# montib/rays1bench

Measured on AMD Instinct MI355X. Metric: mrays/s on 'large' scene 1200x800x10spp, higher is better.
Workload: dtype f32

## Files before the change

### rays1bench_amd/csrc/r1_builds.h

```cpp
#ifndef R1_BUILDS_H
#define R1_BUILDS_H

constexpr int R1_V_REFERENCE = 1;
constexpr int R1_V_SWEEP = 2;
constexpr int R1_V_SWEEP_STATS = 3;
constexpr int R1_V_TREE = 4;
constexpr int R1_V_TREE_STATS = 5;
constexpr int R1_V_WAVEFRONT = 6;
constexpr int R1_V_GRID = 7;
constexpr int R1_V_GRID_STATS = 8;

constexpr int R1_MODE_TP = 0;
constexpr int R1_MODE_LAT = 1;
constexpr int R1_MODE_PIXEL = 2;
constexpr int R1_MODE_BATCH = 3;
constexpr int R1_MODE_PASS = 4;
constexpr int R1_MODE_PATH = 5;
constexpr int R1_MODE_LISTED = 6;
constexpr int R1_MODES = 7;

constexpr bool r1_is_tree(int variant) { return variant == R1_V_TREE || variant == R1_V_TREE_STATS; }
constexpr bool r1_is_grid(int variant) { return variant == R1_V_GRID || variant == R1_V_GRID_STATS; }
constexpr bool r1_is_stats(int variant) { return variant == R1_V_SWEEP_STATS || variant == R1_V_TREE_STATS || variant == R1_V_GRID_STATS; }
constexpr int r1_base_variant(int variant) { return r1_is_stats(variant) ? variant - 1 : variant; }

constexpr bool r1_mode_is_batch(int mode) { return mode == R1_MODE_BATCH || mode == R1_MODE_PATH; }
constexpr bool r1_mode_is_pass(int mode) { return mode == R1_MODE_PASS || mode == R1_MODE_LISTED; }
constexpr bool r1_mode_is_tp_family(int mode) { return mode == R1_MODE_TP || r1_mode_is_batch(mode); }
constexpr bool r1_runs_as_latency(int mode, bool big) { return mode == R1_MODE_LAT || (r1_mode_is_pass(mode) && !big); }
constexpr bool r1_build_lands(int variant, bool stats, int mode) { return variant == R1_V_TREE && !stats && r1_mode_is_tp_family(mode); }

constexpr bool r1_root_by_slots(bool stats, bool big, int mode)
{
    return stats || (mode != R1_MODE_PATH && !(mode == R1_MODE_PIXEL && !big));
}

struct R1Build
{
    int variant;
    bool stats, big;
    int mode;
};

#define R1_BUILDS_TREE_SMALL(X)                 \
    X(R1_V_TREE, false, false, R1_MODE_TP)      \
    X(R1_V_TREE, false, false, R1_MODE_LAT)     \
    X(R1_V_TREE, false, false, R1_MODE_PIXEL)   \
    X(R1_V_TREE, false, false, R1_MODE_BATCH)   \
    X(R1_V_TREE, false, false, R1_MODE_PASS)    \
    X(R1_V_TREE, false, false, R1_MODE_PATH)    \
    X(R1_V_TREE, false, false, R1_MODE_LISTED)  \
    X(R1_V_TREE, true, false, R1_MODE_LAT)
#define R1_BUILDS_TREE_BIG(X)                  \
    X(R1_V_TREE, false, true, R1_MODE_TP)      \
    X(R1_V_TREE, false, true, R1_MODE_PIXEL)   \
    X(R1_V_TREE, false, true, R1_MODE_BATCH)   \
    X(R1_V_TREE, false, true, R1_MODE_PASS)    \
    X(R1_V_TREE, false, true, R1_MODE_PATH)    \
    X(R1_V_TREE, false, true, R1_MODE_LISTED)  \
    X(R1_V_TREE, true, true, R1_MODE_TP)
#define R1_BUILDS_SWEEP_SMALL(X)                   \
    X(R1_V_SWEEP, false, false, R1_MODE_TP)        \
    X(R1_V_SWEEP, false, false, R1_MODE_LAT)       \
    X(R1_V_SWEEP, false, false, R1_MODE_PIXEL)     \
    X(R1_V_SWEEP, false, false, R1_MODE_BATCH)     \
    X(R1_V_SWEEP, false, false, R1_MODE_PASS)      \
    X(R1_V_SWEEP, false, false, R1_MODE_PATH)      \
    X(R1_V_SWEEP, false, false, R1_MODE_LISTED)    \
    X(R1_V_SWEEP, true, false, R1_MODE_LAT)        \
    X(R1_V_REFERENCE, false, false, R1_MODE_TP)    \
    X(R1_V_REFERENCE, false, false, R1_MODE_PASS)
#define R1_BUILDS_SWEEP_BIG(X)   \
    X(R1_V_SWEEP, false, true, R1_MODE_TP)                                         \
    X(R1_V_SWEEP, false, true, R1_MODE_PIXEL)                                      \
    X(R1_V_SWEEP, false, true, R1_MODE_BATCH)                                      \
    X(R1_V_SWEEP, false, true, R1_MODE_PASS)                                       \
    X(R1_V_SWEEP, false, true, R1_MODE_PATH)                                       \
    X(R1_V_SWEEP, false, true, R1_MODE_LISTED)                                     \
    X(R1_V_REFERENCE, false, true, R1_MODE_TP)                                     \
    X(R1_V_REFERENCE, false, true, R1_MODE_PASS)
#define R1_BUILDS_GRID_SMALL(X)                 \
    X(R1_V_GRID, false, false, R1_MODE_TP)      \
    X(R1_V_GRID, false, false, R1_MODE_LAT)     \
    X(R1_V_GRID, false, false, R1_MODE_BATCH)   \
    X(R1_V_GRID, false, false, R1_MODE_PASS)    \
    X(R1_V_GRID, false, false, R1_MODE_PATH)    \
    X(R1_V_GRID, false, false, R1_MODE_LISTED)  \
    X(R1_V_GRID, true, false, R1_MODE_LAT)
#define R1_BUILDS_GRID_BIG(X)                  \
    X(R1_V_GRID, false, true, R1_MODE_TP)      \
    X(R1_V_GRID, false, true, R1_MODE_PIXEL)   \
    X(R1_V_GRID, false, true, R1_MODE_BATCH)   \
    X(R1_V_GRID, false, true, R1_MODE_PASS)    \
    X(R1_V_GRID, false, true, R1_MODE_PATH)    \
    X(R1_V_GRID, false, true, R1_MODE_LISTED)  \
    X(R1_V_GRID, true, true, R1_MODE_TP)
#define R1_BUILDS_ALL(X) R1_BUILDS_TREE_SMALL(X) R1_BUILDS_TREE_BIG(X) R1_BUILDS_SWEEP_SMALL(X) R1_BUILDS_SWEEP_BIG(X) R1_BUILDS_GRID_SMALL(X) R1_BUILDS_GRID_BIG(X)

constexpr bool r1_same_build(const R1Build &a, int variant, bool stats, bool big, int mode)
{
    return a.variant == variant && a.stats == stats && a.big == big && a.mode == mode;
}

constexpr bool r1_build_exists(const R1Build &b)
{
#define R1_X(V, S, B, M) || r1_same_build(b, V, S, B, M)
    return false R1_BUILDS_ALL(R1_X);
#undef R1_X
}

constexpr bool r1_pick(int variant, bool big, int want, R1Build &b)
{
    if (variant < R1_V_REFERENCE || variant > R1_V_GRID_STATS || variant == R1_V_WAVEFRONT || want < 0 || want >= R1_MODES)
        return false;
    const bool single = want == R1_MODE_TP || want == R1_MODE_LAT || want == R1_MODE_PIXEL;
    b.variant = r1_base_variant(variant), b.stats = r1_is_stats(variant), b.big = big, b.mode = want;
    if (b.stats)
    {
        if (!single)
            return false;
        b.mode = big ? R1_MODE_TP : R1_MODE_LAT;
        if (b.variant == R1_V_SWEEP && big)
            b.stats = false;
    }
    else if (variant == R1_V_REFERENCE)
    {
        if (!single && want != R1_MODE_PASS)
            return false;
        b.mode = single ? R1_MODE_TP : R1_MODE_PASS;
    }
    else
    {
        if (want == R1_MODE_LAT && big)
            b.mode = R1_MODE_TP;
        if (variant == R1_V_GRID && want == R1_MODE_PIXEL && !big)
            return false;
    }
    return true;
}

constexpr bool r1_picks_exist()
{
    for (int variant = 0; variant <= 9; ++variant)
        for (int big = 0; big < 2; ++big)
            for (int want = 0; want < R1_MODES; ++want)
            {
                R1Build b = {0, false, false, 0};
                if (r1_pick(variant, big != 0, want, b) && !r1_build_exists(b))
                    return false;
            }
    return true;
}
static_assert(r1_picks_exist(), "r1_pick chose a build that no translation unit instantiates (R1_BUILDS_*)");

#endif
```

### rays1bench_amd/csrc/r1_hit_tree.hpp

```cpp
#ifndef R1_HIT_TREE_HPP
#define R1_HIT_TREE_HPP

#include <hip/hip_runtime.h>
#include <float.h>
#include <stdint.h>

#include "r1_device.h"
#include "r1_exact_math.h"
#include "r1_offer.h"
#include "r1_dev_math.hpp"

#pragma clang fp contract(off)

namespace
{

#define R1_BVH_DONE 0xFFFFFFFFu

__device__ __forceinline__ bool bvh_box(const float mx, const float my, const float mz, const float ex, const float ey, const float ez,
                                        const V3 pa, const V3 oi, const V3 inv, const V3 ainv, const float best, float &t_near)
{
    const float ax = __fmaf_rn(mx, inv.x, -oi.x), ay = __fmaf_rn(my, inv.y, -oi.y), az = __fmaf_rn(mz, inv.z, -oi.z);
    const float bx = __fmaf_rn(ex, ainv.x, pa.x), by = __fmaf_rn(ey, ainv.y, pa.y), bz = __fmaf_rn(ez, ainv.z, pa.z);
    const float tn = fmaxf(fmaxf(ax - bx, ay - by), az - bz);
    const float tf = fminf(fminf(ax + bx, ay + by), az + bz);
    t_near = tn;
    return tn <= tf && tn <= best && tf >= 0.0f;
}

template <int OFFER>
__device__ __forceinline__ void leaf_quad(const float4 *__restrict__ prims, const uint32_t *__restrict__ ids, const uint32_t first,
                                          const uint32_t pairs, const V3 o, const V3 d, float &best, uint32_t &best_id)
{
    float nb[4], ds[4];
#pragma unroll
    for (int h = 0; h < 2; ++h)
    {
        if (h)
            __builtin_amdgcn_sched_barrier(0);
        const float4 p0 = prims[2 * (size_t)first + 2 * h], p1 = prims[2 * (size_t)first + 2 * h + 1];
#pragma unroll
        for (int s = 0; s < 2; ++s)
        {
            const int q = 2 * h + s;
            const float cx = s ? p0.y : p0.x, cy = s ? p0.w : p0.z, cz = s ? p1.y : p1.x, rsq = s ? p1.w : p1.z;
            const float cox = cx - o.x, coy = cy - o.y, coz = cz - o.z;
            nb[q] = __fmaf_rn(coz, d.z, __fmaf_rn(coy, d.y, cox * d.x));
            const float c = __fmaf_rn(coz, coz, __fmaf_rn(coy, coy, cox * cox)) - rsq;
            ds[q] = nb[q] * nb[q] - c;
        }
    }
    uint32_t sgn = __float_as_uint(ds[3]) >> 31;
    sgn = __builtin_amdgcn_alignbit(sgn, __float_as_uint(ds[2]), 31u);
    sgn = __builtin_amdgcn_alignbit(sgn, __float_as_uint(ds[1]), 31u);
    sgn = __builtin_amdgcn_alignbit(sgn, __float_as_uint(ds[0]), 31u);
    uint32_t mask = ~sgn & (pairs < 2u ? 3u : 15u);
    unsigned long long flagged = __builtin_amdgcn_ballot_w64(mask != 0u);
    if (flagged != 0ull)
    do
    {
        const bool have = mask != 0u;
        const uint32_t q = (uint32_t)__builtin_ctz(mask | 8u);
        mask &= mask - 1u;
        const float n_ = q == 0u ? nb[0] : (q == 1u ? nb[1] : (q == 2u ? nb[2] : nb[3]));
        const float d_ = q == 0u ? ds[0] : (q == 1u ? ds[1] : (q == 2u ? ds[2] : ds[3]));
        const uint32_t id = ids[2 * (size_t)first + q];
        const float root = r1_sqrt_exact_lanes(d_, flagged);
        const float t1 = n_ - root;
        const float t = (t1 > 0.001f) ? t1 : n_ + root;
        const bool upd = have & r1_offer_update_form<OFFER>(t, id, best, best_id);
        best = upd ? t : best;
        best_id = upd ? id : best_id;
        flagged = __builtin_amdgcn_ballot_w64(mask != 0u);
    } while (flagged != 0ull);
}

template <int OFFER>
__device__ __forceinline__ void leaf_root(const float4 *__restrict__ prims, const uint32_t *__restrict__ ids, const uint32_t first,
                                          const uint32_t pairs, const V3 o, const V3 d, float &best, uint32_t &best_id)
{
    typedef const uint32_t __attribute__((address_space(4))) *cu32_ptr;
    const cf4_ptr sp = (cf4_ptr)(const f4 *)prims + 2 * (size_t)first;
    const cu32_ptr si = (cu32_ptr)ids + 2 * (size_t)first;
#pragma unroll
    for (int h = 0; h < 2; ++h)
    {
        if (h && pairs < 2u)
            break;
        const f4 p0 = sp[2 * h], p1 = sp[2 * h + 1];
#pragma unroll
        for (int s = 0; s < 2; ++s)
        {
            const float cx = s ? p0.y : p0.x, cy = s ? p0.w : p0.z, cz = s ? p1.y : p1.x, rsq = s ? p1.w : p1.z;
            const float cox = cx - o.x, coy = cy - o.y, coz = cz - o.z;
            const float nb = __fmaf_rn(coz, d.z, __fmaf_rn(coy, d.y, cox * d.x));
            const float c = __fmaf_rn(coz, coz, __fmaf_rn(coy, coy, cox * cox)) - rsq;
            const float ds = nb * nb - c;
            const unsigned long long any = __builtin_amdgcn_ballot_w64((int)__float_as_uint(ds) >= 0);
            if (any != 0ull)
            {
                const bool flag = (int)__float_as_uint(ds) >= 0;
                const uint32_t id = si[2 * h + s];
                const float root = r1_sqrt_exact_lanes(ds, any);
                const float t1 = nb - root;
                const float t = (t1 > 0.001f) ? t1 : nb + root;
                const bool upd = flag & r1_offer_update_form<OFFER>(t, id, best, best_id);
                best = upd ? t : best;
                best_id = upd ? id : best_id;
            }
        }
    }
}

__device__ __forceinline__ void trav_put(uint32_t *trav, const int at, const uint32_t ref) { trav[at] = ref; }
__device__ __forceinline__ uint32_t trav_get(const uint32_t *trav, const int at) { return trav[at]; }
__device__ __forceinline__ void trav_put(uint16_t *trav, const int at, const uint32_t ref) { trav[at] = (uint16_t)ref; }
__device__ __forceinline__ uint32_t trav_get(const uint16_t *trav, const int at) { return trav[at]; }
__device__ __forceinline__ uint32_t r1_ref16(const uint32_t ref) { return ((ref >> 16) & 0xF000u) | (ref & 0x0FFFu); }

struct Trav
{
    uint32_t cur;
    int sp;
    float best;
    uint32_t best_id;
};

__device__ __forceinline__ void trav_start(Trav &t)
{
    t.cur = 0u, t.sp = 0, t.best = FLT_MAX, t.best_id = 0xFFFFFFFFu;
}

#ifndef R1_CARRY_DIV
#define R1_CARRY_DIV 6u
#endif
template <bool STATS, bool CARRY, bool LN, typename TS, bool SLOTS = false, int OFFER = R1_OFFER_FORM>
__device__ __forceinline__ void bvh_advance(const R1DeviceScene &S, const V3 o, const V3 d, Trav &tv, TS *trav, const int tid,
                                            const uint32_t n_alive, unsigned long long *wstat, const float4 *lnodes , const uint32_t top = 0u )
{
    const float4 *__restrict__ nodes = S.bvh_nodes;
    const float4 *__restrict__ prims = S.bvh_prims;
    const uint32_t *__restrict__ ids = S.bvh_ids;
    const V3 inv = mk(__builtin_amdgcn_rcpf(d.x), __builtin_amdgcn_rcpf(d.y), __builtin_amdgcn_rcpf(d.z));
    const V3 ainv = mk(fabsf(inv.x), fabsf(inv.y), fabsf(inv.z));
    V3 oi = mk(o.x * inv.x, o.y * inv.y, o.z * inv.z);
    const float rx = o.x - S.bvh_centre[0], ry = o.y - S.bvh_centre[1], rz = o.z - S.bvh_centre[2];
    const float r2 = __fmaf_rn(rz, rz, __fmaf_rn(ry, ry, rx * rx));
    V3 pa_ray = mk(0.0f, 0.0f, 0.0f);
    if (LN)
    {
        const float pad_ray = lnodes[3].x * r2;
        pa_ray = mk(pad_ray * ainv.x, pad_ray * ainv.y, pad_ray * ainv.z);
    }
    float best = tv.best;
    uint32_t best_id = tv.best_id;
    uint32_t cur = tv.cur;
    int sp = tv.sp;
    constexpr uint32_t LEAF_BIT = LN ? 0x8000u : 0x80000000u, INDEX_MASK = LN ? 0x0FFFu : 0x0FFFFFFFu;
    constexpr int COUNT_SHIFT = LN ? 12 : 28;
    auto visit_node = [&]() {
        if (STATS)
        {
            wstat[9] += 1;
            if ((tid & 63) == __ffsll((long long)__ballot(1)) - 1)
                wstat[2] += 1;
        }
        float4 q0, q1, q2, q3;
        if (LN || cur < top)
        {
            q0 = lnodes[4 * cur + 0], q1 = lnodes[4 * cur + 1], q2 = lnodes[4 * cur + 2], q3 = lnodes[4 * cur + 3];
            if (!LN)
                asm volatile("" : "+v"(q0.x), "+v"(q1.x), "+v"(q2.x), "+v"(q3.x));
        }
        else
            q0 = nodes[4 * (size_t)cur + 0], q1 = nodes[4 * (size_t)cur + 1], q2 = nodes[4 * (size_t)cur + 2],
            q3 = nodes[4 * (size_t)cur + 3];
        float tn0, tn1;
        V3 pa = pa_ray;
        if (!LN)
        {
            float dist2 = r2;
            if (S.bvh_pad_local)
            {
                const float sx = __fmaf_rn(-2.0f, o.x, q0.x + q0.y), sy = __fmaf_rn(-2.0f, o.y, q0.z + q0.w), sz = __fmaf_rn(-2.0f, o.z, q1.x + q1.y);
                dist2 = __fmaf_rn(sz, sz, __fmaf_rn(sy, sy, sx * sx));
            }
            const float pad = __fmaf_rn(q3.x, dist2, q3.y);
            pa = mk(pad * ainv.x, pad * ainv.y, pad * ainv.z);
        }
        const bool h0 = bvh_box(q0.x, q0.z, q1.x, q1.z, q2.x, q2.z, pa, oi, inv, ainv, best, tn0);
        const bool h1 = bvh_box(q0.y, q0.w, q1.y, q1.w, q2.y, q2.w, pa, oi, inv, ainv, best, tn1);
        const uint32_t c0 = __float_as_uint(q3.z), c1 = __float_as_uint(q3.w);
        if (h0 && h1)
        {
            const bool swap = tn1 < tn0;
            trav_put(trav, sp * R1_BLOCK + tid, swap ? c0 : c1);
            ++sp;
            cur = swap ? c1 : c0;
        }
        else if (h0)
            cur = c0;
        else if (h1)
            cur = c1;
        else if (sp > 0)
            cur = trav_get(trav, --sp * R1_BLOCK + tid);
        else
            cur = R1_BVH_DONE;
    };
    auto visit_flat = [&]() {
        if (STATS)
        {
            wstat[9] += 1;
            if ((tid & 63) == __ffsll((long long)__ballot(1)) - 1)
                wstat[2] += 1;
        }
        const float4 q0 = lnodes[4 * cur + 0], q1 = lnodes[4 * cur + 1], q2 = lnodes[4 * cur + 2], q3 = lnodes[4 * cur + 3];
        const float ax0 = __fmaf_rn(q0.x, inv.x, -oi.x), az0 = __fmaf_rn(q1.x, inv.z, -oi.z);
        const float bx0 = __fmaf_rn(q1.z, ainv.x, pa_ray.x), bz0 = __fmaf_rn(q2.z, ainv.z, pa_ray.z);
        const float ax1 = __fmaf_rn(q0.y, inv.x, -oi.x), az1 = __fmaf_rn(q1.y, inv.z, -oi.z);
        const float bx1 = __fmaf_rn(q1.w, ainv.x, pa_ray.x), bz1 = __fmaf_rn(q2.w, ainv.z, pa_ray.z);
        const float tn0 = fmaxf(fmaxf(ax0 - bx0, az0 - bz0), oi.y), tf0 = fminf(fminf(ax0 + bx0, az0 + bz0), pa_ray.y);
        const float tn1 = fmaxf(fmaxf(ax1 - bx1, az1 - bz1), oi.y), tf1 = fminf(fminf(ax1 + bx1, az1 + bz1), pa_ray.y);
        const bool h0 = tn0 <= tf0, h1 = tn1 <= tf1;
        const uint32_t c0 = __float_as_uint(q3.z), c1 = __float_as_uint(q3.w);
        if (h0 && h1)
        {
            const bool swap = tn1 < tn0;
            trav_put(trav, sp * R1_BLOCK + tid, swap ? c0 : c1);
            ++sp;
            cur = swap ? c1 : c0;
        }
        else if (h0)
            cur = c0;
        else if (h1)
            cur = c1;
        else if (sp > 0)
            cur = trav_get(trav, --sp * R1_BLOCK + tid);
        else
            cur = R1_BVH_DONE;
    };
    const uint32_t root_leaf = LN ? __float_as_uint(lnodes[3].y) & 3u : S.bvh_root_leaf;
    if (root_leaf != 0u && cur == 0u)
    {
        const int k = root_leaf == 1u ? 1 : 0;
        const float *nf = (const float *)lnodes;
        const uint32_t leaf = __float_as_uint(nf[14 + (1 - k)]);
        const uint32_t other = __float_as_uint(nf[14 + k]);
        const uint32_t lp = (leaf >> COUNT_SHIFT) & 7u;
        if (STATS)
        {
            wstat[5] += (unsigned long long)lp, wstat[16] += 1ull, wstat[17] += 1ull;
            if ((tid & 63) == __ffsll((long long)__ballot(1)) - 1)
                wstat[3] += 1;
        }
        if (SLOTS)
            leaf_root<OFFER>(prims, ids, (uint32_t)__builtin_amdgcn_readfirstlane((int)(leaf & INDEX_MASK)), (uint32_t)__builtin_amdgcn_readfirstlane((int)lp), o, d, best, best_id);
        else
            leaf_quad<OFFER>(prims, ids, leaf & INDEX_MASK, lp, o, d, best, best_id);
        V3 pa = pa_ray;
        if (!LN)
        {
            float dist2 = r2;
            if (S.bvh_pad_local)
            {
                const float sx = __fmaf_rn(-2.0f, o.x, nf[0] + nf[1]), sy = __fmaf_rn(-2.0f, o.y, nf[2] + nf[3]), sz = __fmaf_rn(-2.0f, o.z, nf[4] + nf[5]);
                dist2 = __fmaf_rn(sz, sz, __fmaf_rn(sy, sy, sx * sx));
            }
            const float pad = __fmaf_rn(nf[12], dist2, nf[13]);
            pa = mk(pad * ainv.x, pad * ainv.y, pad * ainv.z);
        }
        float tn;
        const bool h = bvh_box(nf[0 + k], nf[2 + k], nf[4 + k], nf[6 + k], nf[8 + k], nf[10 + k], pa, oi, inv, ainv, best, tn);
        cur = h ? other : R1_BVH_DONE;
    }
    if (LN && (__builtin_amdgcn_readfirstlane((int)__float_as_uint(lnodes[3].y)) & 4) != 0)
    {
        const float a_u = __fmaf_rn(lnodes[7].x, inv.y, -oi.y), b_u = __fmaf_rn(lnodes[7].y, ainv.y, pa_ray.y);
        const float tyf = a_u + b_u;
        oi.y = fmaxf(a_u - b_u, 0.0f);
        pa_ray.y = tyf < best ? tyf : best;
        cur = oi.y <= pa_ray.y ? cur : R1_BVH_DONE;
    }
    for (;;)
    {
        const unsigned long long walking = __ballot(cur != R1_BVH_DONE);
        if (walking == 0ull)
            break;
        if (CARRY && R1_CARRY_DIV * (uint32_t)__popcll(walking) <= n_alive)
            break;
        if (LN && (__builtin_amdgcn_readfirstlane((int)__float_as_uint(lnodes[3].y)) & 4) != 0)
            while (cur < LEAF_BIT)
                visit_flat();
        else
            while (cur < LEAF_BIT)
                visit_node();
        if (cur != R1_BVH_DONE)
        {
            const uint32_t first = cur & INDEX_MASK, cnt = (cur >> COUNT_SHIFT) & 7u;
            if (LN)
            {
                static_assert(R1_BVH_LEAF <= 4, "the LDS walks test a leaf with ONE leaf_quad call: at most two pairs");
                if (STATS)
                {
                    wstat[5] += (unsigned long long)cnt, wstat[16] += 1ull;
                    if ((tid & 63) == __ffsll((long long)__ballot(1)) - 1)
                        wstat[3] += 1;
                }
                leaf_quad<OFFER>(prims, ids, first, cnt, o, d, best, best_id);
            }
            else
            for (uint32_t j = 0; j < cnt; j += 2u)
            {
                const uint32_t take = cnt - j < 2u ? 1u : 2u;
                if (STATS)
                {
                    wstat[5] += (unsigned long long)take;
                    wstat[16] += 1ull;
                    if ((tid & 63) == __ffsll((long long)__ballot(1)) - 1)
                        wstat[3] += 1;
                }
                leaf_quad<OFFER>(prims, ids, first + j, take, o, d, best, best_id);
            }
            cur = sp > 0 ? trav_get(trav, --sp * R1_BLOCK + tid) : R1_BVH_DONE;
            if (LN && (__builtin_amdgcn_readfirstlane((int)__float_as_uint(lnodes[3].y)) & 4) != 0)
                pa_ray.y = best < pa_ray.y ? best : pa_ray.y;
        }
    }
    tv.cur = cur, tv.sp = sp, tv.best = best, tv.best_id = r1_offer_settle_form<OFFER>(best, best_id);
}

template <bool STATS>
__device__ __forceinline__ void sweep_bvh(const R1DeviceScene &S, const bool alive, const V3 o, const V3 d, float &t_max, int &hit_index,
                                          uint32_t *trav, const int tid, unsigned long long *wstat)
{
    Trav tv;
    trav_start(tv);
    if (!alive)
        tv.cur = R1_BVH_DONE;
    bvh_advance<STATS, false, false, uint32_t>(S, o, d, tv, trav, tid, 64u, wstat, nullptr);
    if (tv.best_id != 0xFFFFFFFFu)
    {
        t_max = tv.best;
        hit_index = (int)tv.best_id;
    }
}

}

#endif
```

### rays1bench_amd/csrc/r1_trace.hpp

```cpp
#ifndef R1_TRACE_HPP
#define R1_TRACE_HPP

#include <hip/hip_runtime.h>
#include <float.h>
#include <stdint.h>

#include "r1_device.h"
#include "r1_dev_math.hpp"
#include "r1_kargs.hpp"
#include "r1_hit_sweep.hpp"
#include "r1_hit_tree.hpp"
#include "r1_hit_grid.hpp"
#include "r1_sample.hpp"
#include "r1_shade.hpp"
#include "r1_land.hpp"

#pragma clang fp contract(off)

template <int VARIANT, bool STATS, bool BIG, int MODE>
struct TraceWaves
{
#ifndef R1_TREE_WAVES_TP
#define R1_TREE_WAVES_TP 7
#endif
#ifndef R1_TREE_WAVES_LAT
#define R1_TREE_WAVES_LAT 6
#endif
    static constexpr int value = STATS ? 1 : (VARIANT == R1_V_GRID && MODE == R1_MODE_PIXEL) ? 4 : ((r1_is_tree(VARIANT) || r1_is_grid(VARIANT)) ? (BIG ? 8 : (r1_mode_is_tp_family(MODE) ? R1_TREE_WAVES_TP : R1_TREE_WAVES_LAT)) : (VARIANT == R1_V_SWEEP && !BIG ? 5 : 1));
};

template <int VARIANT, bool STATS, bool BIG, int MODE>
__device__ __forceinline__ void r1_trace_body(const R1TraceArgs A)
{
    constexpr bool LISTED = MODE == R1_MODE_LISTED, PASS = r1_mode_is_pass(MODE);
    constexpr bool CPATH = MODE == R1_MODE_PATH, BATCH = r1_mode_is_batch(MODE);
    constexpr bool LAT = r1_runs_as_latency(MODE, BIG), PIX = MODE == R1_MODE_PIXEL;
    constexpr bool LAND = r1_build_lands(VARIANT, STATS, MODE);
    const uint32_t tb = blockIdx.x, n_tb = gridDim.x;
    const uint32_t xcd = LAND ? (uint32_t)__builtin_amdgcn_readfirstlane((int)(xcc_id() & (R1_LAND_MAX_XCD - 1u))) : 0u;
    const uint32_t land_tiles = LAND ? A.total_samples / A.full : 0u;
#ifdef R1_LAND_DEBUG
    if (LAND && threadIdx.x == 0 && blockIdx.x < 8)
        A.queue[R1_HEAD_WORDS * (R1_HEAD_DEBUG + blockIdx.x % R1_HEAD_DEBUG_COUNT)] = 0x1000u | (xcc_id() << 4) | xcd;
#endif
    if (LAND && blockIdx.x == 0)
        for (uint32_t i = threadIdx.x; i < R1_HEAD_WORDS * A.land.clear_count; i += R1_BLOCK)
            A.land.clear_heads[i] = 0u;
    typedef typename IdxType<BIG>::type IDX;
    unsigned long long wstat[18];
    if (STATS)
    {
        for (int i = 0; i < 18; ++i)
            wstat[i] = 0;
        wstat[14] = __builtin_readcyclecounter();
    }
    unsigned long long *wave_log = nullptr;
    unsigned long long log_start = 0, log_exhausted = 0;
    if (STATS && A.stats)
    {
        wave_log = (unsigned long long *)A.stats[R1_STATS_WORDS];
        log_start = __builtin_amdgcn_s_memrealtime();
    }
    constexpr int LW = (r1_is_tree(VARIANT) || r1_is_grid(VARIANT)) ? ((r1_mode_is_tp_family(MODE) && !STATS) ? R1_STACK_LDS_WORDS_TP : R1_STACK_LDS_WORDS) : R1_STACK_WORDS;
    __shared__ uint32_t s_stack[BIG ? 1 : LW * R1_BLOCK];
    __shared__ uint32_t s_cand[VARIANT == R1_V_SWEEP ? (BIG ? R1_CAND_CAP : R1_BIT_WORDS) * R1_BLOCK : 1];
    __shared__ IDX s_pairs[VARIANT == R1_V_SWEEP ? (R1_BLOCK / 64) * PairBits<IDX>::cap : 1];
    extern __shared__ uint32_t s_trav[];
    const uint32_t gstride = n_tb * R1_BLOCK, gtid = tb * R1_BLOCK + threadIdx.x;
    __shared__ unsigned long long s_best[VARIANT == R1_V_SWEEP ? R1_BLOCK : 1];
    __shared__ f4 s_tile[BIG && VARIANT == R1_V_SWEEP ? 2 * R1_TILE_F4 : 1];

    const int tid = (int)threadIdx.x;
    const int lane = tid & 63;

    constexpr bool LN = VARIANT == R1_V_TREE && !BIG;
    typedef typename IdxType<!LN>::type TS;
    const size_t trav_words = VARIANT == R1_V_TREE ? (size_t)A.bvh_depth * R1_BLOCK * sizeof(TS) / 4 : 0;
    const size_t gtrav_words = VARIANT == R1_V_GRID ? (size_t)A.bvh_depth * R1_BLOCK : 0;
    const uint16_t *ltab = (const uint16_t *)(s_trav + gtrav_words);
    if (VARIANT == R1_V_GRID && !BIG)
    {
        float4 *dst = (float4 *)(s_trav + gtrav_words);
        const R1GridCArgs *ga = (const R1GridCArgs *)(uintptr_t)A.grid;
        const float4 *src = (const float4 *)(const r1_gu32 *)ga->tab;
        const uint32_t n16 = ga->lds_bytes / 16u;
        for (uint32_t i = (uint32_t)tid; i < n16; i += R1_BLOCK)
            dst[i] = src[i];
        __syncthreads();
    }
    const float4 *lnodes = (const float4 *)(s_trav + trav_words);
    const uint32_t top = LN ? 0u : A.bvh_lds_f4 >> 2;
    if (VARIANT == R1_V_TREE && A.bvh_lds_f4)
    {
        float4 *dst = (float4 *)(s_trav + trav_words);
        for (uint32_t i = (uint32_t)tid; i < A.bvh_lds_f4; i += R1_BLOCK)
        {
            float4 q = A.scene.bvh_nodes[i];
            if (LN && (i & 3u) == 3u)
                q.z = __uint_as_float(r1_ref16(__float_as_uint(q.z))), q.w = __uint_as_float(r1_ref16(__float_as_uint(q.w)));
            dst[i] = q;
        }
        if (LN && tid == 3)
            ((float *)dst)[13] = __uint_as_float(A.scene.bvh_root_leaf | (A.scene.bvh_flat_e >= 0.0f ? 4u : 0u));
        if (LN && tid == 7 && A.scene.bvh_flat_e >= 0.0f)
            ((float *)dst)[28] = A.scene.bvh_flat_m, ((float *)dst)[29] = A.scene.bvh_flat_e;
        __syncthreads();
    }

    Path p;
    p.o = mk(0, 0, 0), p.d = mk(0, 0, 0);
    p.s_scalar = p.s0 = p.s1 = p.s2 = 1;
    p.k = 0, p.depth = 0, p.sp = 0;
    bool alive = false;
    Pixel px;
    px.acc = mk(0, 0, 0), px.xy = 0, px.off = 0, px.s = (uint32_t)A.spp;
    Trav tv;
    trav_start(tv);
    tv.cur = R1_BVH_DONE;
    unsigned long long lane_rays = 0;
#ifndef R1_SPARE_MIN
#define R1_SPARE_MIN 40u
#endif
    constexpr bool SPARE = !BIG && (VARIANT == R1_V_TREE || VARIANT == R1_V_SWEEP || VARIANT == R1_V_GRID) && r1_mode_is_tp_family(MODE);
    Path spare = p;
    bool has_spare = false;
    constexpr bool TRIM = LAND && SPARE;
#ifndef R1_TRIM_VOTES
#define R1_TRIM_VOTES 1
#endif
#ifndef R1_TRIM_WALK
#define R1_TRIM_WALK 1
#endif
    constexpr bool TRIM_VOTES = TRIM && R1_TRIM_VOTES, TRIM_WALK = TRIM && R1_TRIM_WALK;
#define R1_DEAD (TRIM_VOTES ? tv.cur == R1_BVH_DONE : !alive)
#define R1_VOTE(c) (TRIM_VOTES ? (unsigned long long)__builtin_amdgcn_ballot_w64(c) : (unsigned long long)__ballot(c))

    uint32_t q_next = 0, q_end = 0;
    const uint32_t q_total = A.total_samples;
    uint32_t q_remaining = q_total;
    const uint32_t n_waves2 = 2u * n_tb * (R1_BLOCK / 64);
    uint32_t *const q_head = LAND ? A.queue + R1_HEAD_WORDS * (R1_HEAD_XCD + xcd) : A.queue;
    constexpr uint32_t LAND_GROUP = LAT ? 8u : 1u;
    __shared__ uint32_t s_land[LAND ? (R1_BLOCK / 64) * R1_LAND_ROW : 1];
#define row (s_land + (LAND ? (threadIdx.x >> 6) * R1_LAND_ROW : 0u))
    if (LAND && lane < 8)
        row[lane] = (lane == 0 || lane == 2) ? 0xFFFFFFFFu : 0u;
    bool exhausted = false;
    const uint32_t home = LAT && A.nq > 1 ? __builtin_amdgcn_readfirstlane(((tb >> 3) * (R1_BLOCK / 64) + (threadIdx.x >> 6)) % A.nq) : 0u;

    for (;;)
    {
        if (STATS)
            wstat[15] = __builtin_readcyclecounter();
        if (PIX && !alive && px.s < (uint32_t)A.spp)
        {
            start_ray(A, A.cam, p, (int)(px.xy & 0xFFFFu), (int)(px.xy >> 16), px.s, A.seed);
            alive = true;
            if (VARIANT == R1_V_TREE)
                trav_start(tv);
        }
        if (SPARE && R1_DEAD && has_spare)
        {
            p.o = spare.o, p.d = spare.d, p.s_scalar = spare.s_scalar, p.s0 = spare.s0, p.s1 = spare.s1, p.s2 = spare.s2, p.k = spare.k;
            p.depth = 0, p.sp = 0;
            alive = true, has_spare = false;
            if (TRIM_WALK)
                tv.cur = 0u;
            else
                trav_start(tv);
        }
        unsigned long long need = R1_VOTE(R1_DEAD);
        if (SPARE)
        {
            const unsigned long long lack = R1_VOTE(!has_spare);
            const uint32_t n_lack = TRIM_VOTES ? (uint32_t)__builtin_popcount((uint32_t)lack) + (uint32_t)__builtin_popcount((uint32_t)(lack >> 32)) : (uint32_t)__popcll(lack);
            need = (need != 0ull || n_lack >= R1_SPARE_MIN) ? lack : 0ull;
        }
        while (need)
        {
            if (q_next == q_end)
            {
                if (exhausted)
                    break;
                uint32_t want, base = 0;
                if (LAT && A.nq > 1)
                {
                    want = A.chunk_max;
                    if (lane == 0)
                        base = atomicAdd(A.queue + R1_HEAD_WORDS * (R1_HEAD_SUBQUEUE + home), 1u);
                    base = (__builtin_amdgcn_readfirstlane(base) * A.nq + home) * want;
                }
                else if (LAND)
                {
                    want = min(A.chunk_max, max(A.chunk_min, q_remaining / n_waves2));
                    base = q_total;
                    for (;;)
                    {
                        unsigned long long old = 0;
                        if (lane == 0)
                            old = __hip_atomic_fetch_add((unsigned long long *)q_head, (unsigned long long)want, __ATOMIC_RELAXED, __HIP_MEMORY_SCOPE_AGENT);
                        const uint32_t hi = (uint32_t)__builtin_amdgcn_readfirstlane((int)(uint32_t)(old >> 32));
                        const uint32_t lo = (uint32_t)__builtin_amdgcn_readfirstlane((int)(uint32_t)old);
                        if (hi == 0xFFFFFFFFu)
                            break;
                        const uint32_t g0 = (hi - 1u) * LAND_GROUP;
                        const uint32_t gs = hi != 0u ? min(LAND_GROUP, land_tiles - g0) * A.full : 0u;
                        const bool have = hi != 0u && lo < gs;
                        const bool advance = (hi == 0u && lo == 0u) || (have && lo + want >= gs);
                        if (advance && lane == 0)
                        {
                            const uint32_t g = __hip_atomic_fetch_add(A.queue + R1_HEAD_WORDS * R1_HEAD_DISPENSER, 1u, __ATOMIC_RELAXED, __HIP_MEMORY_SCOPE_AGENT);
                            unsigned long long nv = 0xFFFFFFFFull << 32;
                            if (g * LAND_GROUP < land_tiles)
                                nv = (unsigned long long)(g + 1u) << 32;
                            (void)__hip_atomic_exchange((unsigned long long *)q_head, nv, __ATOMIC_RELAXED, __HIP_MEMORY_SCOPE_AGENT);
                        }
                        if (have)
                        {
                            base = g0 * A.full + lo;
                            want = min(want, gs - lo);
                            q_remaining = (land_tiles - min(land_tiles, g0 + LAND_GROUP)) * A.full;
                            const uint32_t tl = fastdiv(lo, A.div_full);
                            if (lane == 0)
                            {
                                land_chunk(A, row, g0 + tl);
                                if (lo - tl * A.full + want > A.full)
                                    land_chunk(A, row, g0 + tl + 1u);
                            }
                            break;
                        }
                        if (advance)
                            continue;
                        for (;;)
                        {
                            __builtin_amdgcn_s_sleep(16);
                            unsigned long long now = 0;
                            if (lane == 0)
                                now = __hip_atomic_load((unsigned long long *)q_head, __ATOMIC_RELAXED, __HIP_MEMORY_SCOPE_AGENT);
                            if ((uint32_t)__builtin_amdgcn_readfirstlane((int)(uint32_t)(now >> 32)) != hi)
                                break;
                        }
                    }
                }
                else
                {
                    want = min(A.chunk_max, max(A.chunk_min, q_remaining / n_waves2));
                    if (lane == 0)
                        base = atomicAdd(q_head, want);
                    base = __builtin_amdgcn_readfirstlane(base);
                }
                if (base >= q_total)
                {
                    exhausted = true;
                    if (STATS)
                        log_exhausted = __builtin_amdgcn_s_memrealtime();
                    break;
                }
                q_next = base;
                q_end = min(base + want, q_total);
                if (!LAND)
                    q_remaining = q_total - q_end;
            }
            const uint32_t avail = q_end - q_next;
            const uint32_t rank = __builtin_amdgcn_mbcnt_hi((uint32_t)(need >> 32), __builtin_amdgcn_mbcnt_lo((uint32_t)need, 0u));
            R1ArgWords FA_words;
            if (!PIX)
                fresh_args(FA_words);
            const R1TraceArgs &FA = PIX ? A : FA_words.a;
            if (SPARE)
            {
                if (!has_spare && rank < avail)
                    has_spare = start_sample<BATCH, PASS, CPATH, LISTED>(FA, spare, q_next + rank);
            }
            else if (!alive && rank < avail)
            {
                if (PIX)
                {
                    alive = pixel_take(A, px, q_next + rank);
                    if (alive)
                        start_ray(A, A.cam, p, (int)(px.xy & 0xFFFFu), (int)(px.xy >> 16), 0u, A.seed);
                }
                else
                    alive = start_sample<BATCH, PASS, CPATH, LISTED>(FA, p, q_next + rank);
                if (VARIANT == R1_V_TREE && alive)
                    trav_start(tv);
            }
            q_next += min((uint32_t)__popcll(need), avail);
            need = SPARE ? R1_VOTE(!has_spare) : R1_VOTE(!alive);
        }
        if (SPARE && R1_DEAD && has_spare)
        {
            p.o = spare.o, p.d = spare.d, p.s_scalar = spare.s_scalar, p.s0 = spare.s0, p.s1 = spare.s1, p.s2 = spare.s2, p.k = spare.k;
            p.depth = 0, p.sp = 0;
            alive = true, has_spare = false;
            if (TRIM_WALK)
                tv.cur = 0u;
            else
                trav_start(tv);
        }
        if (BIG && VARIANT == R1_V_SWEEP)
        {
            if (!__syncthreads_or(alive ? 1 : 0))
                break;
        }
        else if (!TRIM_VOTES && __ballot(alive) == 0ull)
            break;
        if (TRIM_VOTES)
            alive = !R1_DEAD;
        const unsigned long long live_once = TRIM_VOTES ? (unsigned long long)__builtin_amdgcn_ballot_w64(!R1_DEAD) : 0ull;
        if (TRIM_VOTES && live_once == 0ull)
            break;
        if (TRIM_VOTES)
        {
            if ((__builtin_amdgcn_ballot_w64(p.depth >= 12) & live_once) == 0ull)
                __builtin_amdgcn_s_setprio(0);
            else if ((__builtin_amdgcn_ballot_w64(p.depth >= 36) & live_once) != 0ull)
                __builtin_amdgcn_s_setprio(3);
            else if ((__builtin_amdgcn_ballot_w64(p.depth >= 24) & live_once) != 0ull)
                __builtin_amdgcn_s_setprio(2);
            else
                __builtin_amdgcn_s_setprio(1);
        }
        else
        {
            if (__ballot(alive && p.depth >= 12) == 0ull)
                __builtin_amdgcn_s_setprio(0);
            else if (__ballot(alive && p.depth >= 36) != 0ull)
                __builtin_amdgcn_s_setprio(3);
            else if (__ballot(alive && p.depth >= 24) != 0ull)
                __builtin_amdgcn_s_setprio(2);
            else
                __builtin_amdgcn_s_setprio(1);
        }
        if (STATS)
        {
            wstat[4] += __builtin_readcyclecounter() - wstat[15];
            wstat[15] = __builtin_readcyclecounter();
            wstat[0] += 1;
            wstat[1] += (unsigned long long)__popcll(__ballot(alive));
        }

        float t_hit = FLT_MAX;
        int hit = -1;
        bool ready = alive;
        const unsigned long long live_now = TRIM_VOTES ? live_once : __ballot(alive);
        if (LAT && !BIG && VARIANT != R1_V_REFERENCE && exhausted && (uint32_t)__popcll(live_now) <= A.coop_lanes)
        {
            cooperative_sweep(A.scene, live_now, p.o, p.d, t_hit, hit, lane);
            tv.cur = R1_BVH_DONE;
        }
        else if (VARIANT == R1_V_REFERENCE)
        {
            if (alive)
                sweep_reference(A.scene, p.o, p.d, t_hit, hit);
        }
        else if (VARIANT == R1_V_TREE)
        {
            R1_FRESH_ARGS(HA)
            bvh_advance<STATS, true, LN, TS, r1_root_by_slots(STATS, BIG, MODE)>(HA.scene, p.o, p.d, tv, (TS *)s_trav, tid, (uint32_t)__popcll(live_now), wstat, lnodes, top);
            ready = alive && tv.cur == R1_BVH_DONE;
            if (tv.best_id != 0xFFFFFFFFu)
                t_hit = tv.best, hit = (int)tv.best_id;
        }
        else if (VARIANT == R1_V_GRID)
        {
            R1_FRESH_ARGS(HA)
            float best;
            uint32_t best_id;
            const bool fb = grid_trace<STATS, !BIG>(HA, (R1GridCArgs *)(uintptr_t)HA.grid, alive, p.o, p.d, best, best_id, ltab, tid, wstat);
            if (STATS)
                wstat[16] += fb ? 1ull : 0ull;
            if (__ballot(fb) != 0ull)
            {
                Trav fv;
                trav_start(fv);
                fv.best = best, fv.best_id = best_id;
                if (!fb)
                    fv.cur = R1_BVH_DONE;
                bvh_advance<false, false, false, uint32_t, false, R1_OFFER_FORM_GRID>(HA.scene, p.o, p.d, fv, s_trav, tid, 64u, wstat, nullptr);
                best = fv.best, best_id = fv.best_id;
            }
            if (best_id != 0xFFFFFFFFu)
                t_hit = best, hit = (int)best_id;
        }
        else
        {
            R1ArgWords HA_words;
            if (!PIX)
                fresh_args(HA_words);
            const R1TraceArgs &HA = PIX ? A : HA_words.a;
            sweep_prefilter<STATS, IDX, BIG>(HA.scene, alive, p.o, p.d, t_hit, hit, s_cand, s_pairs, s_best, s_tile, tid, wstat);
        }
        if (STATS)
        {
            wstat[6] += __builtin_readcyclecounter() - wstat[15];
            wstat[15] = __builtin_readcyclecounter();
        }

        bool fin = false;
        R1ArgWords SA_words;
        if (!PIX)
            fresh_args(SA_words);
        const R1TraceArgs &SA = PIX ? A : SA_words.a;
        if (ready)
        {
            V3 col;
            if (shade_level<BIG, LW>(SA, p, hit, t_hit, s_stack, gstride, gtid, tid, col))
            {
                if (PIX)
                {
                    px.acc = vadd(px.acc, col);
                    if (++px.s == (uint32_t)SA.spp)
                        pixel_write(SA, px);
                }
                else if (LAND)
                    SA.samples[p.k] = make_float4(col.x, col.y, col.z, __uint_as_float(path_rays(p) | SA.land_tag));
                else
                    SA.samples[p.k] = make_float4(col.x, col.y, col.z, __uint_as_float(path_rays(p)));
                if (!LAND)
                    lane_rays += path_rays(p);
                alive = false, fin = true;
            }
            else if (VARIANT == R1_V_TREE && !TRIM_WALK)
                trav_start(tv);
            if (TRIM_WALK)
            {
                trav_start(tv);
                if (fin)
                    tv.cur = R1_BVH_DONE;
            }
        }
        if (LAND && fin)
            land_count(SA, row, p.k);
        if (STATS)
            wstat[7] += __builtin_readcyclecounter() - wstat[15];
    }
    if (STATS)
    {
        wstat[8] = __builtin_readcyclecounter() - wstat[14];
        unsigned long long c9 = wstat[9];
        for (int off = 32; off > 0; off >>= 1)
            c9 += __shfl_down(c9, off, 64);
        wstat[9] = c9;
        if (VARIANT == R1_V_TREE || VARIANT == R1_V_GRID)
        {
            const int slots[5] = {2, 3, 5, 16, 17};
            for (int q = 0; q < 5; ++q)
            {
                unsigned long long c = wstat[slots[q]];
                for (int off = 32; off > 0; off >>= 1)
                    c += __shfl_down(c, off, 64);
                wstat[slots[q]] = c;
            }
        }
        if (lane == 0 && wave_log)
        {
            unsigned long long *rec = wave_log + 4 * (size_t)(blockIdx.x * (R1_BLOCK / 64) + (threadIdx.x >> 6));
            if (VARIANT == R1_V_GRID)
            {
                typedef unsigned long long __attribute__((address_space(1))) gu64;
                gu64 *grec = (gu64 *)(uintptr_t)rec;
                grec[0] = log_start, grec[1] = log_exhausted, grec[2] = __builtin_amdgcn_s_memrealtime(), grec[3] = wstat[0];
            }
            else
                rec[0] = log_start, rec[1] = log_exhausted, rec[2] = __builtin_amdgcn_s_memrealtime(), rec[3] = wstat[0];
        }
        if (lane == 0 && A.stats)
        {
            for (int i = 0; i < 10; ++i)
                atomicAdd(&A.stats[i], wstat[i]);
            atomicMax(&A.stats[10], wstat[8]);
            atomicMax(&A.stats[11], ~wstat[8]);
            atomicMax(&A.stats[12], (unsigned long long)__builtin_readcyclecounter());
            atomicMax(&A.stats[13], ~wstat[14]);
            if (VARIANT == R1_V_TREE || VARIANT == R1_V_GRID)
            {
                atomicAdd(&A.stats[14], wstat[16]);
                atomicAdd(&A.stats[15], wstat[17]);
            }
        }
    }

    if (LAND)
        land_exit<(BIG && VARIANT == R1_V_TREE) ? 6 : R1_LAND_LOADS>(A, row, lane);
#undef row
#undef R1_VOTE
#undef R1_DEAD
    if (!LAND)
    {
        for (int off = 32; off > 0; off >>= 1)
            lane_rays += __shfl_down(lane_rays, off, 64);
        if (lane == 0 && lane_rays)
            atomicAdd(A.num_rays, lane_rays);
    }
}

template <int VARIANT, bool STATS, bool BIG, int MODE>
__global__ void __launch_bounds__(R1_BLOCK, (TraceWaves<VARIANT, STATS, BIG, MODE>::value)) r1_trace_kernel(const R1TraceArgs A)
{
    r1_trace_body<VARIANT, STATS, BIG, MODE>(A);
}

template <bool STATS, bool BIG, int MODE>
__global__ void __launch_bounds__(R1_BLOCK, (TraceWaves<R1_V_GRID, STATS, BIG, MODE>::value)) r1_grid_kernel(const R1TraceArgs A)
{
    r1_trace_body<R1_V_GRID, STATS, BIG, MODE>(A);
}

template <int VARIANT, bool BIG>
__global__ void __launch_bounds__(R1_BLOCK, (TraceWaves<VARIANT, false, BIG, R1_MODE_PASS>::value)) r1_pass_kernel(const R1TraceArgs A)
{
    r1_trace_body<VARIANT, false, BIG, R1_MODE_PASS>(A);
}

template <int VARIANT, bool BIG>
__global__ void __launch_bounds__(R1_BLOCK, (TraceWaves<VARIANT, false, BIG, R1_MODE_PASS>::value)) r1_adaptive_kernel(const R1TraceArgs A)
{
    r1_trace_body<VARIANT, false, BIG, R1_MODE_LISTED>(A);
}

template <int VARIANT, bool BIG>
__global__ void __launch_bounds__(R1_BLOCK, (TraceWaves<VARIANT, false, BIG, R1_MODE_PATH>::value)) r1_path_kernel(const R1TraceArgs A)
{
    r1_trace_body<VARIANT, false, BIG, R1_MODE_PATH>(A);
}

#endif
```

Before: 44140.

## Add vote-driven BVH walk choosing node or leaf steps per wave

Adds a voted traversal loop for the tree walker. Each iteration the wave ballots how many lanes sit on inner nodes versus leaves and picks a node step or a leaf step by a weighted majority rule, instead of draining all inner nodes before any lane tests leaves. It is enabled by default only for big TP/batch builds. The goal is to cut SIMD divergence where lanes idle while others finish node walks, at the cost of two extra ballots per step and a carry-exit check that now runs only after leaf steps.

Result: no change. 44100, median of 2 (-0.1%).

```diff
diff --git a/rays1bench_amd/csrc/r1_builds.h b/rays1bench_amd/csrc/r1_builds.h
--- a/rays1bench_amd/csrc/r1_builds.h
+++ b/rays1bench_amd/csrc/r1_builds.h
@@ -33,6 +33,17 @@
 constexpr bool r1_root_by_slots(bool stats, bool big, int mode)
 {
     return stats || (mode != R1_MODE_PATH && !(mode == R1_MODE_PIXEL && !big));
+}
+
+#if !defined(R1_TUNING) || !defined(R1_WALK_VOTED_BUILDS)
+#undef R1_WALK_VOTED_BUILDS
+#define R1_WALK_VOTED_BUILDS 8
+#endif
+constexpr bool r1_walk_voted(bool stats, bool big, int mode)
+{
+    return stats ? (R1_WALK_VOTED_BUILDS & 1) != 0
+                 : (mode == R1_MODE_TP || mode == R1_MODE_BATCH) ? (R1_WALK_VOTED_BUILDS & (big ? 8 : 2)) != 0
+                                                                 : mode == R1_MODE_PATH && !big && (R1_WALK_VOTED_BUILDS & 4) != 0;
 }
 
 struct R1Build
diff --git a/rays1bench_amd/csrc/r1_hit_tree.hpp b/rays1bench_amd/csrc/r1_hit_tree.hpp
--- a/rays1bench_amd/csrc/r1_hit_tree.hpp
+++ b/rays1bench_amd/csrc/r1_hit_tree.hpp
@@ -8,6 +8,7 @@
 #include "r1_device.h"
 #include "r1_exact_math.h"
 #include "r1_offer.h"
+#include "r1_walk_rule.h"
 #include "r1_dev_math.hpp"
 
 #pragma clang fp contract(off)
@@ -134,7 +135,7 @@
 #ifndef R1_CARRY_DIV
 #define R1_CARRY_DIV 6u
 #endif
-template <bool STATS, bool CARRY, bool LN, typename TS, bool SLOTS = false, int OFFER = R1_OFFER_FORM>
+template <bool STATS, bool CARRY, bool LN, typename TS, bool SLOTS = false, int OFFER = R1_OFFER_FORM, bool VOTED = false>
 __device__ __forceinline__ void bvh_advance(const R1DeviceScene &S, const V3 o, const V3 d, Trav &tv, TS *trav, const int tid,
                                             const uint32_t n_alive, unsigned long long *wstat, const float4 *lnodes , const uint32_t top = 0u )
 {
@@ -281,6 +282,72 @@
         pa_ray.y = tyf < best ? tyf : best;
         cur = oi.y <= pa_ray.y ? cur : R1_BVH_DONE;
     }
+    auto visit_leaf = [&]() {
+        const uint32_t first = cur & INDEX_MASK, cnt = (cur >> COUNT_SHIFT) & 7u;
+        if (LN)
+        {
+            static_assert(R1_BVH_LEAF <= 4, "the LDS walks test a leaf with ONE leaf_quad call: at most two pairs");
+            if (STATS)
+            {
+                wstat[5] += (unsigned long long)cnt, wstat[16] += 1ull;
+                if ((tid & 63) == __ffsll((long long)__ballot(1)) - 1)
+                    wstat[3] += 1;
+            }
+            leaf_quad<OFFER>(prims, ids, first, cnt, o, d, best, best_id);
+        }
+        else
+        for (uint32_t j = 0; j < cnt; j += 2u)
+        {
+            const uint32_t take = cnt - j < 2u ? 1u : 2u;
+            if (STATS)
+            {
+                wstat[5] += (unsigned long long)take;
+                wstat[16] += 1ull;
+                if ((tid & 63) == __ffsll((long long)__ballot(1)) - 1)
+                    wstat[3] += 1;
+            }
+            leaf_quad<OFFER>(prims, ids, first + j, take, o, d, best, best_id);
+        }
+        cur = sp > 0 ? trav_get(trav, --sp * R1_BLOCK + tid) : R1_BVH_DONE;
+        if (LN && (__builtin_amdgcn_readfirstlane((int)__float_as_uint(lnodes[3].y)) & 4) != 0)
+            pa_ray.y = best < pa_ray.y ? best : pa_ray.y;
+    };
+    if (VOTED)
+    {
+        auto vote = [&](const bool after_leaf) -> int {
+            const unsigned long long walking = __builtin_amdgcn_ballot_w64(cur != R1_BVH_DONE);
+            const unsigned long long on_node = __builtin_amdgcn_ballot_w64(cur < LEAF_BIT);
+            const uint32_t n_node = (uint32_t)__popcll(on_node), n_leaf = (uint32_t)__popcll(walking & ~on_node);
+            if (walking == 0ull)
+                return 0;
+            if (CARRY && r1_walk_exit_tested(R1_WALK_EXIT, after_leaf, n_leaf) && r1_walk_carry_exit(n_node + n_leaf, n_alive, R1_CARRY_DIV))
+                return 0;
+            return r1_walk_node_step(n_node, n_leaf) ? 1 : 2;
+        };
+        for (;;)
+        {
+            int step = vote(true);
+            if (LN && (__builtin_amdgcn_readfirstlane((int)__float_as_uint(lnodes[3].y)) & 4) != 0)
+                while (step == 1)
+                {
+                    if (cur < LEAF_BIT)
+                        visit_flat();
+                    step = vote(false);
+                }
+            else
+                while (step == 1)
+                {
+                    if (cur < LEAF_BIT)
+                        visit_node();
+                    step = vote(false);
+                }
+            if (step == 0)
+                break;
+            if (!(cur < LEAF_BIT) && cur != R1_BVH_DONE)
+                visit_leaf();
+        }
+    }
+    else
     for (;;)
     {
         const unsigned long long walking = __ballot(cur != R1_BVH_DONE);
@@ -299,7 +366,6 @@
             const uint32_t first = cur & INDEX_MASK, cnt = (cur >> COUNT_SHIFT) & 7u;
             if (LN)
             {
-                static_assert(R1_BVH_LEAF <= 4, "the LDS walks test a leaf with ONE leaf_quad call: at most two pairs");
                 if (STATS)
                 {
                     wstat[5] += (unsigned long long)cnt, wstat[16] += 1ull;
diff --git a/rays1bench_amd/csrc/r1_trace.hpp b/rays1bench_amd/csrc/r1_trace.hpp
--- a/rays1bench_amd/csrc/r1_trace.hpp
+++ b/rays1bench_amd/csrc/r1_trace.hpp
@@ -357,7 +357,7 @@
         else if (VARIANT == R1_V_TREE)
         {
             R1_FRESH_ARGS(HA)
-            bvh_advance<STATS, true, LN, TS, r1_root_by_slots(STATS, BIG, MODE)>(HA.scene, p.o, p.d, tv, (TS *)s_trav, tid, (uint32_t)__popcll(live_now), wstat, lnodes, top);
+            bvh_advance<STATS, true, LN, TS, r1_root_by_slots(STATS, BIG, MODE), R1_OFFER_FORM, r1_walk_voted(STATS, BIG, MODE)>(HA.scene, p.o, p.d, tv, (TS *)s_trav, tid, (uint32_t)__popcll(live_now), wstat, lnodes, top);
             ready = alive && tv.cur == R1_BVH_DONE;
             if (tv.best_id != 0xFFFFFFFFu)
                 t_hit = tv.best, hit = (int)tv.best_id;
diff --git a/rays1bench_amd/csrc/r1_walk_rule.h b/rays1bench_amd/csrc/r1_walk_rule.h
--- /dev/null
+++ b/rays1bench_amd/csrc/r1_walk_rule.h
@@ -0,0 +1,43 @@
+#ifndef R1_WALK_RULE_H
+#define R1_WALK_RULE_H
+
+#include <stdint.h>
+
+#if defined(__HIPCC__)
+#include <hip/hip_runtime.h>
+#define R1_WALK_HD __host__ __device__ __forceinline__
+#else
+#define R1_WALK_HD inline
+#endif
+
+#ifndef R1_WALK_NUM
+#define R1_WALK_NUM 2u
+#endif
+#ifndef R1_WALK_DEN
+#define R1_WALK_DEN 1u
+#endif
+#ifndef R1_WALK_EXIT
+#define R1_WALK_EXIT 1
+#endif
+
+R1_WALK_HD bool r1_walk_node_step_weighted(const uint32_t n_node, const uint32_t n_leaf, const uint32_t num, const uint32_t den)
+{
+    return n_node > 0u && (unsigned long long)num * n_node >= (unsigned long long)den * n_leaf;
+}
+
+R1_WALK_HD bool r1_walk_node_step(const uint32_t n_node, const uint32_t n_leaf)
+{
+    return r1_walk_node_step_weighted(n_node, n_leaf, R1_WALK_NUM, R1_WALK_DEN);
+}
+
+R1_WALK_HD bool r1_walk_carry_exit(const uint32_t walking, const uint32_t n_alive, const uint32_t carry_div)
+{
+    return carry_div * walking <= n_alive;
+}
+
+R1_WALK_HD bool r1_walk_exit_tested(const int where, const bool after_leaf, const uint32_t n_leaf)
+{
+    return where == 0 ? true : (where == 1 ? after_leaf : n_leaf == 0u);
+}
+
+#endif
```
